# aszepieniec/stark-brainfuck

Hardware: AMD Instinct MI355X
Metric: goldilocks_ntt_field_elements_per_sec (higher is better)
Workload: dtype u64 (mod 2^64-2^32+1)

## Files before the change

### stark_brainfuck_amd/_lib.py

```python
import ctypes
import os

_HERE = os.path.dirname(os.path.abspath(__file__))
LIB_PATH = os.environ.get("BFS_LIB_PATH") or os.path.join(_HERE, "libbfstark_hip.so")

u64 = ctypes.c_uint64
u32 = ctypes.c_uint32
vp = ctypes.c_void_p
sz = ctypes.c_size_t
ci = ctypes.c_int

BFS_OK = 0
ASSERT_CODES = {1, 2, 3, 4, 5, 8, 9}

_SIGNATURES = {
    "bfs_version": (ci, []),
    "bfs_last_error": (ctypes.c_char_p, []),
    "bfs_device_count": (ci, [ctypes.POINTER(ci)]),
    "bfs_set_device": (ci, [ci]),
    "bfs_malloc": (ci, [ctypes.POINTER(vp), sz]),
    "bfs_free": (ci, [vp]),
    "bfs_malloc_async": (ci, [ctypes.POINTER(vp), sz, vp]),
    "bfs_free_async": (ci, [vp, vp]),
    "bfs_pool_trim": (ci, []),
# ... 132 lines not shown
    "bfs_stark_verify_finish": (ci, [vp, vp, ctypes.POINTER(u64), u32, ctypes.POINTER(ci)]),
    "bfs_stark_verify_finish_fri": (ci, [vp, vp, ctypes.POINTER(u64), u32, u32, ci, u32, ctypes.POINTER(ci)]),
    "bfs_stark_session_set_fri": (ci, [vp, u32, ci, u32]),
    "bfs_stark_session_new": (vp, []),
    "bfs_stark_session_free": (None, [vp]),
    "bfs_stark_commit": (ci, [vp, vp, vp, vp, vp, ctypes.POINTER(u64), ctypes.POINTER(u64), ctypes.POINTER(u64), ctypes.POINTER(ctypes.c_double), vp]),
    "bfs_stark_finish": (ci, [vp, vp, ctypes.POINTER(u64), ctypes.POINTER(u64), ctypes.POINTER(u64), u32, ctypes.c_int32, ctypes.POINTER(u64), u32,
                              ctypes.POINTER(u64), vp, ctypes.POINTER(u64), ctypes.POINTER(ctypes.c_double), vp]),
}

_EXT_SIGNATURES = {
    "bfs_poly_eval_points": (ci, [vp, u64, u64, u32, ctypes.POINTER(u64), u32, vp, vp]),
    "bfs_deep_quotient": (ci, [vp, u32, u64, u32, u64, u64, ctypes.POINTER(u64), ctypes.POINTER(u64), u32, ctypes.POINTER(u64), vp, u64, vp]),
}

_OPEN_SIGNATURES = {
    "bfsx_poly_eval_columns": (ci, [vp, u32, ctypes.POINTER(u64), u32, vp, vp]),
    "bfsx_deep_quotient_groups": (ci, [vp, u32, u64, u32, u64, u64, ctypes.POINTER(u32), ctypes.POINTER(u32), u32, ctypes.POINTER(u64), u32,
                                       ctypes.POINTER(u32), ctypes.POINTER(u64), ctypes.POINTER(u64), vp, u64, vp]),
}

_ROUNDS_SIGNATURES = {
    "bfsr_deep_quotient_rounds": (ci, [vp, u32, u64, u32, u64, u64, ctypes.POINTER(u32), ctypes.POINTER(u32), u32, ctypes.POINTER(u64), u32,
                                       ctypes.POINTER(u32), ctypes.POINTER(u64), ctypes.POINTER(u64), vp, u64, ctypes.POINTER(u32), vp]),
}


_COMPOSE_SIGNATURES = {
    "bfsc_air_compose": (ci, [ci, vp, vp, u32, u64, u64, u64, u64, u64, ctypes.POINTER(u64), ctypes.POINTER(u64), ctypes.POINTER(u64), ctypes.POINTER(u64),
                              u32, ci, vp, vp]),
    "bfsc_difference_compose": (ci, [vp, vp, u32, u64, u64, ctypes.POINTER(u64), u32, ci, vp, vp]),
}


class GatherRequest(ctypes.Structure):
    _fields_ = [("d_base", vp), ("nwords", u32), ("stride", u32), ("out_offset", u64)]


class AirViolation(ctypes.Structure):
    _fields_ = [("first_row", u64), ("count", u64)]


class RowColumn(ctypes.Structure):
    _fields_ = [("d_values", vp), ("is_ext", ctypes.c_int32), ("field_id", ctypes.c_int32)]


class EvalColumn(ctypes.Structure):
    _fields_ = [("d_coeffs", vp), ("n_coeffs", u64)]


class TracePadTable(ctypes.Structure):
    _fields_ = [("d_rows", vp), ("rows", u64), ("row_stride", u64), ("height", u64), ("d_out", vp), ("d_mask0", vp), ("d_mask1", vp),
                ("d_mask2", vp), ("kind", ctypes.c_int32), ("width", u32)]


class CombSource(ctypes.Structure):
    _fields_ = [("ptr", vp), ("is_ext", u32), ("pad", u32), ("shift", u64), ("wa", u64 * 3), ("wb", u64 * 3)]

class ScanSpec(ctypes.Structure):
    _fields_ = [("kind", ctypes.c_int32), ("record_before", ctypes.c_int32), ("d_x1", vp), ("d_x2", vp), ("d_x3", vp), ("shift1", u64),
                ("d_mask", vp), ("n", u64), ("constants", u64 * 12), ("initial", u64 * 3), ("d_out", vp), ("out_stride", u64),
                ("d_terminal", vp)]


class StarkParams(ctypes.Structure):
    _fields_ = [("log_n", u32), ("expansion_factor", u32), ("num_colinearity_checks", u32), ("security_level", u32), ("offset", u64),
# ... 14 lines not shown
    _fields_ = [("randomizer_seed", vp), ("randomizer_limbs", vp), ("base_randomizers", vp), ("base_salt_seed", vp), ("base_salts", vp),
                ("initials", u64 * 6), ("ext_randomizers", vp), ("ext_salt_seed", vp), ("ext_salts", vp)]


class CombWeight(ctypes.Structure):
    _fields_ = [("wa", u64 * 3), ("wb", u64 * 3), ("shift", u64)]


_lib = None


class BackendUnavailable(RuntimeError):
    pass


def exported_symbols():
    return sorted(_SIGNATURES)


def ext_exported_symbols():
    return sorted(_EXT_SIGNATURES)


def open_exported_symbols():
    return sorted(_OPEN_SIGNATURES)


def rounds_exported_symbols():
    return sorted(_ROUNDS_SIGNATURES)


def compose_exported_symbols():
    return sorted(_COMPOSE_SIGNATURES)


def load():
    global _lib
    if _lib is not None:
        return _lib
    if not os.path.exists(LIB_PATH):
        raise BackendUnavailable(
            "libbfstark_hip.so is not built (%s). Run `python -m stark_brainfuck_amd.build`; "
            "there is no CPU fallback for the hot path." % LIB_PATH)
    try:
        import torch
    except ImportError:
        pass
    lib = ctypes.CDLL(LIB_PATH)
    for name, (res, args) in (list(_SIGNATURES.items()) + list(_EXT_SIGNATURES.items()) + list(_OPEN_SIGNATURES.items()) + list(_ROUNDS_SIGNATURES.items())
                              + list(_COMPOSE_SIGNATURES.items())):
        fn = getattr(lib, name)
        fn.restype = res
        fn.argtypes = args
    _lib = lib
    return lib


def check(rc):
    if rc == BFS_OK:
        return
    msg = load().bfs_last_error().decode("utf-8", "replace")
    if rc in ASSERT_CODES:
        raise AssertionError(msg)
    raise RuntimeError("libbfstark_hip: error %d: %s" % (rc, msg))
```

### stark_brainfuck_amd/csrc/fri.hip

```cpp
#include <algorithm>
#include <chrono>
#include <map>
#include <unordered_map>
#include <vector>

#include "../../include/bfstark.h"
#include "blake2b.hpp"
#include "refpickle.hpp"
#include "runtime.hpp"

namespace bfs {

template <int K>
__global__ void __launch_bounds__(K == 1 ? 1024 : 256) fri_fold_kernel(FriFoldArgs f, u64* out, u64 out_stride) {
    for (u64 i = (u64)blockIdx.x * blockDim.x + threadIdx.x; i < f.half; i += (u64)gridDim.x * blockDim.x) {
        const Xfe r = fri_fold_point<K>(f, i);
        out[i] = r.c[0];
        out[out_stride + i] = r.c[1];
        out[2 * out_stride + i] = r.c[2];
    }
}

constexpr u32 FRI_FOLD_GRID_MAX = 4096;
static int fri_fold_launch(const FriFoldArgs& f, u64* out, u64 out_stride, hipStream_t stream) {
// ... 19 lines not shown
}

static int gather_run(const std::vector<GatherReq>& reqs, u64 nwords, hipStream_t stream, PinnedLease& req_area, PinnedLease& res_area, const u64** words) {
    BFS_TRY(req_area.get(reqs.size() * sizeof(GatherReq)));
    BFS_TRY(res_area.get(nwords * sizeof(u64)));
    memcpy(req_area.host, reqs.data(), reqs.size() * sizeof(GatherReq));
    hipLaunchKernelGGL(gather_requests_kernel, dim3((u32)((reqs.size() + 255) / 256)), dim3(256), 0, stream, (const GatherReq*)req_area.dev, (u32)reqs.size(),
                       (u64*)res_area.dev);
    BFS_HIP(hipGetLastError());
    BFS_HIP(hipStreamSynchronize(stream));
    *words = (const u64*)res_area.host;
    return BFS_OK;
}

static thread_local double g_fri_timing[8] = {0, 0, 0, 0, 0, 0, 0, 0};
static inline double now_ms() { return std::chrono::duration<double, std::milli>(std::chrono::steady_clock::now().time_since_epoch()).count(); }

enum class TreePath : unsigned char {
    Borrowed,
    Coset,
    OneLaunch,
    FoldInLeaves,
    Codeword,
    SingleElement,
};

struct FriRound {
    const u64* cw = nullptr;
    u64 stride = 0, length = 0;
    u64 leaves = 0;
    u64* nodes = nullptr;
    TreePath path = TreePath::Codeword;
    unsigned char root[64];
};

struct RootMailbox {
    u64* host = nullptr;
    u64* dev = nullptr;
    u64 seq = 0;
    int init() {
        if (host) return BFS_OK;
        BFS_TRY(host_alloc(16 * sizeof(u64), (void**)&host));
        memset(host, 0, 16 * sizeof(u64));
        BFS_HIP(hipHostGetDevicePointer((void**)&dev, host, 0));
        return BFS_OK;
    }
    ~RootMailbox() { if (host) (void)host_release(host); }
};

struct FriSession {
    std::vector<FriRound> rounds;
    void* block = nullptr;
    bool use_workspace = false;
    RootMailbox mailbox;
    u32 log_n = 0;
    u32 log2_folding = 1;
    bool coset_leaves = false;
    u32 grinding_bits = 0;
    u64 grinding_window = POW_DEFAULT_WINDOW;
    u64 round0_leaves = 0;
    struct Key {
        u64 v;
        Key(u32 round, u64 index) : v(((u64)round << 48) | index) {}
        bool operator==(const Key& o) const { return v == o.v; }
    };
    struct KeyMap {
        std::vector<u64> keys;
        std::vector<u32> slots;
        std::vector<rp::Ref> vals;
        void reserve(size_t n) { size_t cap = 64; while (cap < 2 * n) cap <<= 1; if (cap > keys.size()) rehash(cap); vals.reserve(n); }
        void rehash(size_t cap) {
            std::vector<u64> k2(cap, 0);
            std::vector<u32> s2(cap, 0);
            for (size_t i = 0; i < keys.size(); ++i)
                if (keys[i]) { size_t j = slot_of(keys[i], cap); while (k2[j]) j = (j + 1) & (cap - 1); k2[j] = keys[i]; s2[j] = slots[i]; }
            keys.swap(k2); slots.swap(s2);
        }
        static size_t slot_of(u64 stored, size_t cap) { return (size_t)((stored * 0x9E3779B97F4A7C15ULL) >> 20) & (cap - 1); }
        size_t find(const Key& key) const {
            size_t j = slot_of(key.v + 1, keys.size());
// ... 62 lines not shown
        p = (u64*)w;
    } else {
        if (S.block) { (void)device_release(S.block, S.block_stream); S.block = nullptr; }
        BFS_TRY(device_alloc(words * sizeof(u64), stream, &S.block));
        S.block_stream = stream;
        p = (u64*)S.block;
    }
    for (u32 r = 0; r < R; ++r) {
        FriRound& fr = S.rounds[r];
        fr.nodes = p; p += 16 * fr.leaves;
        if (r == 0) { fr.cw = d_cw; fr.stride = stride; }
        else { fr.cw = p; fr.stride = fr.length; p += 3 * fr.length; }
    }
    return S.mailbox.init();
}

static int launch_round_tree(FriSession& S, u32 r, const FriFoldArgs& fold, hipStream_t stream, u64* seq) {
    FriRound& fr = S.rounds[r];
    const bool folds = fold.in != nullptr;
    u64* const cw = (u64*)fr.cw;
    u64* const box = S.mailbox.dev;
    *seq = 0;
    if (folds != (r >= 1)) { set_error("internal: round %u of the plan and its fold disagree", r); return BFS_ERR_BAD_ARG; }
    switch (fr.path) {
    case TreePath::Borrowed:
        fr.nodes = (u64*)S.round0_nodes;
        memcpy(fr.root, S.round0_root, 64);
        return BFS_OK;
    case TreePath::SingleElement:
        if (folds) BFS_TRY(fri_fold_launch(fold, cw, fr.stride, stream));
        return merkle_build_xfe_launch(fr.cw, fr.stride, fr.length, fr.nodes, stream);
    case TreePath::Coset:
        *seq = ++S.mailbox.seq;
        return coset_tree_launch(folds ? &fold : nullptr, cw, fr.stride, fr.leaves, S.log2_folding, fr.nodes, stream, box + 9, *seq, box, *seq);
    case TreePath::OneLaunch:
        *seq = ++S.mailbox.seq;
        return fri_round_fused_launch(fold, cw, fr.stride, fr.length, fr.nodes, stream, box, *seq);
    case TreePath::FoldInLeaves:
        *seq = ++S.mailbox.seq;
        return merkle_build_xfe_fold_launch(fold, cw, fr.stride, fr.length, fr.nodes, stream, box, *seq);
    case TreePath::Codeword:
        *seq = ++S.mailbox.seq;
        return merkle_build_xfe_launch(fr.cw, fr.stride, fr.length, fr.nodes, stream, box, *seq);
    }
    set_error("internal: round %u has no tree path", r);
    return BFS_ERR_BAD_ARG;
}

int fri_commit(FriSession& S, rp::Transcript& ps, const u64* d_cw, u64 stride, u32 log_n, u64 offset, u64 omega,
               u32 expansion, hipStream_t stream) {
    const double t_begin = now_ms();
    BFS_TRY(plan_rounds(S, d_cw, stride, log_n, omega, expansion, stream));
    const u32 k = S.log2_folding;
    const u32 R = (u32)S.rounds.size();
    const u64 *winv_lo = nullptr, *winv_hi = nullptr;
    u32 lo_bits = 0;
    BFS_TRY(ntt_power_tables(gl_inv(omega), log_n, &winv_lo, &winv_hi, &lo_bits));
    u64 g = offset, w = omega;
    FriFoldArgs fold{};
    rp::Transcript::Lookahead look;
    static const bool lookahead_on = getenv("BFS_FRI_LOOKAHEAD") == nullptr || atoi(getenv("BFS_FRI_LOOKAHEAD")) != 0;
    static const bool trace = getenv("BFS_FRI_TRACE") != nullptr;
    bool looking = false, look_begun = false;
    auto begin_lookahead = [&]() {
        if (look_begun) return;
        look_begun = true;
        const double t_look = trace ? now_ms() : 0;
        looking = lookahead_on && R >= 3 && ps.lookahead_begin(look, R - 2);
        if (trace) fprintf(stderr, "fri look-ahead %s: %.1f us, %zu objects in front\n", looking ? "on" : "off", 1e3 * (now_ms() - t_look), ps.objects.size());
    };
    for (u32 r = 0; r < R; ++r) {
        FriRound& fr = S.rounds[r];
        unsigned char seed[32];
        bool have_seed = false, speculating = false;
        const double t_round = trace ? now_ms() : 0;
        double t_launched = 0, t_absorbed = 0, t_root = 0;
        rp::Transcript::Speculation speculation;
        auto await_root = [&](u64 seq) -> int {
            if (trace) t_launched = now_ms();
            if (r >= 1) begin_lookahead();
            if (r + 1 < R) {
                if (r == 0) { ps.fiat_shamir(ps.objects.size(), seed, 32); have_seed = true; }
                else if (!looking) { ps.speculate(speculation); speculating = true; }
            }
            if (trace) t_absorbed = now_ms();
            volatile u64* flag = S.mailbox.host + 8;
            u64 spins = 0;
            while (__atomic_load_n(flag, __ATOMIC_ACQUIRE) != seq) {
                if (++spins > (1ull << 22)) {
                    BFS_HIP(hipStreamSynchronize(stream));
                    if (__atomic_load_n(flag, __ATOMIC_ACQUIRE) != seq) { set_error("root mailbox was not written"); return BFS_ERR_HIP; }
                    break;
                }
            }
            memcpy(fr.root, S.mailbox.host, 64);
            return BFS_OK;
        };
        u64 seq = 0;
        BFS_TRY(launch_round_tree(S, r, fold, stream, &seq));
        if (seq != 0) {
            BFS_TRY(await_root(seq));
            if (fr.path == TreePath::Coset && __atomic_load_n(S.mailbox.host + 9, __ATOMIC_ACQUIRE) == seq) {
                BFS_TRY(coset_tree_rows(fr.cw, fr.stride, fr.leaves, k, fr.nodes, fr.root, stream));
            }
        } else if (fr.path == TreePath::SingleElement) {
            if (r >= 1) begin_lookahead();
            BFS_HIP(hipMemcpyAsync(fr.root, fr.nodes + 8, 64, hipMemcpyDeviceToHost, stream));
            BFS_HIP(hipStreamSynchronize(stream));
        }
        if (trace) t_root = now_ms();
        if (speculating) ps.resolve(speculation, fr.root, seed, 32);
        else if (r > 0 && looking) { ps.lookahead_next(look, fr.root, r + 1 < R ? seed : nullptr, 32); have_seed = r + 1 < R; }
        else if (r > 0) ps.objects.push_back(rp::mk_bytes(fr.root, 64));
        if (trace)
            fprintf(stderr, "fri round %2u  n %8llu  launch %6.1f us  absorb %6.1f us  wait %6.1f us  finish %6.1f us\n", r, (unsigned long long)fr.length,
                    1e3 * (t_launched - t_round), 1e3 * (t_absorbed - t_launched), 1e3 * (t_root - t_absorbed), 1e3 * (now_ms() - t_root));
        if (r == R - 1) break;
        if (!speculating && !have_seed) ps.fiat_shamir(ps.objects.size(), seed, 32);
        fold.in = fr.cw; fold.in_stride = fr.stride;
        fold.winv_lo = winv_lo; fold.winv_hi = winv_hi; fold.lo_bits = lo_bits; fold.round_shift = k * r;
        fri_fold_constants(fold, k, fr.length, rp::sample_xfe(seed, 32), g, w);
        for (u32 j = 0; j < k; ++j) { g = gl_sqr(g); w = gl_sqr(w); }
    }
    g_fri_timing[0] = now_ms() - t_begin;
    FriRound& last = S.rounds[R - 1];
    std::vector<u64> host(3 * last.length);
    if (last.stride == last.length) {
        BFS_HIP(hipMemcpyAsync(host.data(), last.cw, 3 * last.length * sizeof(u64), hipMemcpyDeviceToHost, stream));
    } else {
        for (int k = 0; k < 3; ++k)
            BFS_HIP(hipMemcpyAsync(host.data() + k * last.length, last.cw + k * last.stride, last.length * sizeof(u64), hipMemcpyDeviceToHost, stream));
    }
    BFS_HIP(hipStreamSynchronize(stream));
    std::vector<rp::Ref> items;
    for (u64 j = 0; j < last.length; ++j) {
// ... 480 lines not shown
```

### stark_brainfuck_amd/csrc/merkle.hip

```cpp
#include "blake2b_quad.hpp"
#include "merkle_core.hpp"
#include <vector>

#include "runtime.hpp"

namespace bfs {

constexpr int LEAF_THREADS = 64;

constexpr int LEAF_STAGE_WORDS = XFE_STREAM_WORDS * LEAF_THREADS;

__device__ __forceinline__ void xfe_leaves_wave(u64 c0, u64 c1, u64 c2, bool active, u64* stage , u64 h[8], const u64* midstates) {
    const u32 lane = threadIdx.x;
    const u32 k = active ? xfe_leaf_k(c0, c1, c2) : 0u;
    if (active && k == 0) merkle_leaf_xfe_zero(h, midstates);
    if (__ballot(k == 3) != 0) { if (k == 3) merkle_leaf_xfe_stream<3>(c0, c1, c2, stage + lane, LEAF_THREADS, h, midstates); }
    if (__ballot(k == 2) != 0) { if (k == 2) merkle_leaf_xfe_stream<2>(c0, c1, c2, stage + lane, LEAF_THREADS, h, midstates); }
    if (__ballot(k == 1) != 0) { if (k == 1) merkle_leaf_xfe_stream<1>(c0, c1, c2, stage + lane, LEAF_THREADS, h, midstates); }
}

__device__ __forceinline__ void xfe_leaves_wave_store(u64 c0, u64 c1, u64 c2, bool active, u64* stage, u64* leaf_digests, u64 i, const u64* midstates) {
    u64 d[8];
    xfe_leaves_wave(c0, c1, c2, active, stage, d, midstates);
    if (!active) return;
    u64* out = leaf_digests + i * 8;
#pragma unroll
    for (int j = 0; j < 8; ++j) out[j] = d[j];
}

__global__ void __launch_bounds__(LEAF_THREADS) merkle_leaves_xfe_kernel(const u64* limbs, u64 limb_stride, u64 n, u64* leaf_digests, const u64* midstates) {
    __shared__ u64 stage[LEAF_STAGE_WORDS];
    const u64 i = (u64)blockIdx.x * LEAF_THREADS + threadIdx.x;
    const bool active = i < n;
    u64 c0 = 0, c1 = 0, c2 = 0;
// ... 21 lines not shown

__global__ void __launch_bounds__(LEAF_THREADS) merkle_leaves_bfe_kernel(const u64* values, u64 n, u64* leaf_digests) {
    __shared__ u64 stage[BFE_LEAF_MAX_WORDS * LEAF_THREADS];
    const u64 i = (u64)blockIdx.x * LEAF_THREADS + threadIdx.x;
    if (i >= n) return;
    u64 d[8];
    merkle_leaf_bfe_body(values, i, stage + threadIdx.x, LEAF_THREADS, d);
    u64* out = leaf_digests + i * 8;
#pragma unroll
    for (int j = 0; j < 8; ++j) out[j] = d[j];
}

__global__ void blake2b_batch_kernel(const u64* data, const u64* offsets, const u32* lengths, u64 n, u64* digests) {
    const u64 i = (u64)blockIdx.x * blockDim.x + threadIdx.x;
    if (i >= n) return;
    u64 h[8];
    blake2b_staged<true>(data + offsets[i], 1, lengths[i], h);
    u64* out = digests + i * 8;
#pragma unroll
    for (int j = 0; j < 8; ++j) out[j] = h[j];
}

__global__ void merkle_parents_kernel(u64* nodes, u64 first, u64 count, u64 present_children) {
    const u64 t = (u64)blockIdx.x * blockDim.x + threadIdx.x;
    if (t >= count) return;
    const u64 k = first + t;
    const u64 c = 2 * t;
    int present = c + 1 < present_children ? 2 : (c < present_children ? 1 : 0);
    u64 out[8];
    merkle_parent_body(nodes + (2 * k) * 8, nodes + (2 * k + 1) * 8, present, out);
    u64* dst = nodes + k * 8;
#pragma unroll
    for (int j = 0; j < 8; ++j) dst[j] = out[j];
}

__global__ void __launch_bounds__(256) merkle_top_kernel(u64* nodes, u32 width, u64 present_children, u64* root_out, u64 seq) {
    __shared__ u64 lvl[512 * 8];
    const u32 t = threadIdx.x;
    for (u32 i = t; i < 2 * width * 8; i += 256) lvl[i] = nodes[(u64)2 * width * 8 + i];
    __syncthreads();
    u64 present = present_children;
    for (u32 w = width; w >= 1; w >>= 1) {
        u64 out[8];
        if (t < w) {
            const u64 c = 2 * (u64)t;
            int pr = c + 1 < present ? 2 : (c < present ? 1 : 0);
            merkle_parent_body(lvl + (2 * t) * 8, lvl + (2 * t + 1) * 8, pr, out);
        }
        __syncthreads();
        if (t < w) {
            u64* dst = nodes + ((u64)w + t) * 8;
#pragma unroll
            for (int j = 0; j < 8; ++j) { lvl[t * 8 + j] = out[j]; dst[j] = out[j]; }
            if (w == 1 && root_out != nullptr) {
#pragma unroll
                for (int j = 0; j < 8; ++j) __hip_atomic_store(root_out + j, out[j], __ATOMIC_RELAXED, __HIP_MEMORY_SCOPE_SYSTEM);
                __hip_atomic_store(root_out + 8, seq, __ATOMIC_RELEASE, __HIP_MEMORY_SCOPE_SYSTEM);
            }
        }
        __syncthreads();
        present = 2 * (u64)w;
    }
}


__global__ void __launch_bounds__(256) merkle_parents_quad_kernel(u64* nodes, u64 first, u64 count, u64 present_children) {
#if defined(__HIP_DEVICE_COMPILE__)
    __shared__ u64 msg[64 * 16];
    const u32 q = threadIdx.x >> 2, j = threadIdx.x & 3;
    const u64 t = (u64)blockIdx.x * 64 + q;
    const QuadLane ql = quad_lane(threadIdx.x);
    if (t < count) {
        const u64 k = first + t, c = 2 * t;
        const int present = c + 1 < present_children ? 2 : (c < present_children ? 1 : 0);
        const u64* child = nodes + (2 * k) * 8;
#pragma unroll
        for (int w = 0; w < 4; ++w) {
            const int idx = 4 * j + w;
            msg[q * 16 + idx] = (idx < 8 * present) ? child[idx] : 0;
        }
        u64 hl, hh;
        blake2b_init_quad(ql, hl, hh);
        blake2b_compress_quad(ql, hl, hh, msg + q * 16, (u64)(64 * present + 32 * (2 - present)), true);
        nodes[k * 8 + j] = hl;
        nodes[k * 8 + 4 + j] = hh;
    }
#endif
}

#if defined(__HIP_DEVICE_COMPILE__)
__device__ __forceinline__ void quad_parent(const QuadLane& ql, const u64* m, u64 bytes, u64& hl, u64& hh) {
    blake2b_init_quad(ql, hl, hh);
    blake2b_compress_quad(ql, hl, hh, m, bytes, true);
}
__device__ __forceinline__ void quad_parent_store(u32 j, u64 hl, u64 hh, u64* dst, u64* g) {
    dst[j] = hl;
    dst[4 + j] = hh;
    g[j] = hl;
    g[4 + j] = hh;
}

constexpr int QUAD_LEAF_WORDS = 48;

__device__ __forceinline__ void xfe_leaf_quad(u64 c0, u64 c1, u64 c2, u64* m, const QuadLane& ql, u32 j, const u64* midstates, u64& hl, u64& hh) {
    const u32 k = xfe_leaf_k(c0, c1, c2);
    if (k == 0) {
        hl = midstates[(size_t)2 * LEAF_MS_LEN * 8 + j];
        hh = midstates[(size_t)2 * LEAF_MS_LEN * 8 + 4 + j];
    } else {
        const u32 body = xfe_leaf_body_len(k, c0, c1, c2), total = body + 11;
        const u32 nblk = (total + 127) / 128;
        const u64* ms = midstates + ((size_t)(k == 1 ? 0 : 1) * LEAF_MS_LEN + body) * 8;
        hl = ms[j];
        hh = ms[4 + j];
        if (j == 0) {
            LeafWriter w;
            w.init(m, 1);
            encode_xfe_leaf_tail(w, k, c0, c1, c2);
            for (u32 x = w.wpos; x < (nblk - 1) * 16; ++x) m[x] = 0;
        }
        for (u32 b = 1; b < nblk; ++b) {
            const bool last = b + 1 == nblk;
            blake2b_compress_quad(ql, hl, hh, m + 16 * (b - 1), last ? (u64)total : (u64)(b + 1) * 128, last);
        }
    }
}
#endif

__global__ void __launch_bounds__(1024) merkle_top_quad_kernel(u64* nodes, u32 width, u64 present_children, u64* root_out, u64 seq) {
#if defined(__HIP_DEVICE_COMPILE__)
    __shared__ u64 bufA[512 * 8];
    __shared__ u64 bufB[256 * 8];
    const u32 tid = threadIdx.x, q = tid >> 2, j = tid & 3;
    const QuadLane ql = quad_lane(tid);
    for (u32 i = tid; i < 2 * width * 8; i += 1024) bufA[i] = nodes[(u64)2 * width * 8 + i];
    __syncthreads();
    u64* src = bufA;
    u64* dst = bufB;
    u64 present = present_children;
    for (u32 w = width; w >= 1; w >>= 1) {
        if (q < w) {
            const u64 c = 2 * (u64)q;
            const int pr = c + 1 < present ? 2 : (c < present ? 1 : 0);
            u64* m = src + q * 16;
            if (pr < 2) {
#pragma unroll
                for (int wd = 0; wd < 4; ++wd) { const int idx = 4 * j + wd; if (idx >= 8 * pr) m[idx] = 0; }
            }
            u64 hl, hh;
            quad_parent(ql, m, (u64)(64 * pr + 32 * (2 - pr)), hl, hh);
            quad_parent_store(j, hl, hh, dst + q * 8, nodes + ((u64)w + q) * 8);
            if (w == 1 && root_out != nullptr) {
                __hip_atomic_store(root_out + j, hl, __ATOMIC_RELAXED, __HIP_MEMORY_SCOPE_SYSTEM);
                __hip_atomic_store(root_out + 4 + j, hh, __ATOMIC_RELAXED, __HIP_MEMORY_SCOPE_SYSTEM);
            }
        }
        __syncthreads();
        u64* tmp = src; src = dst; dst = tmp;
        present = 2 * (u64)w;
    }
    if (tid == 0 && root_out != nullptr) {
        __threadfence_system();
        __hip_atomic_store(root_out + 8, seq, __ATOMIC_RELEASE, __HIP_MEMORY_SCOPE_SYSTEM);
    }
#endif
}

__global__ void __launch_bounds__(1024) merkle_subtree_quad_kernel(u64* nodes, u64 children) {
#if defined(__HIP_DEVICE_COMPILE__)
    __shared__ u64 bufA[512 * 8];
    __shared__ u64 bufB[256 * 8];
    const u32 tid = threadIdx.x, q = tid >> 2, j = tid & 3;
    const QuadLane ql = quad_lane(tid);
    const u64* in = nodes + (children + (u64)blockIdx.x * 512) * 8;
    for (u32 i = tid; i < 512 * 8; i += 1024) bufA[i] = in[i];
    __syncthreads();
    u64* src = bufA;
    u64* dst = bufB;
    u64 level = children >> 1;
    for (u32 w = 256; w >= 1; w >>= 1, level >>= 1) {
        if (q < w) {
            u64 hl, hh;
            quad_parent(ql, src + q * 16, 128, hl, hh);
            quad_parent_store(j, hl, hh, dst + q * 8, nodes + (level + (u64)blockIdx.x * w + q) * 8);
        }
        __syncthreads();
        u64* tmp = src; src = dst; dst = tmp;
    }
#endif
}

__global__ void __launch_bounds__(256) merkle_leaves_xfe_quad_kernel(const u64* limbs, u64 limb_stride, u64 n, u64* leaf_digests, const u64* midstates) {
#if defined(__HIP_DEVICE_COMPILE__)
    __shared__ u64 stage[64 * QUAD_LEAF_WORDS];
    const u32 q = threadIdx.x >> 2, j = threadIdx.x & 3;
    const u64 i = (u64)blockIdx.x * 64 + q;
    const QuadLane ql = quad_lane(threadIdx.x);
    if (i >= n) return;
    u64* m = stage + q * QUAD_LEAF_WORDS;
    const u64 c0 = limbs[i], c1 = limbs[limb_stride + i], c2 = limbs[2 * limb_stride + i];
    u64 hl, hh;
    xfe_leaf_quad(c0, c1, c2, m, ql, j, midstates, hl, hh);
    leaf_digests[i * 8 + j] = hl;
    leaf_digests[i * 8 + 4 + j] = hh;
#endif
}

constexpr u32 FRI_WG_LEAVES = 64;

template <int K>
__global__ void __launch_bounds__(4 * FRI_WG_LEAVES) fri_round_quad_kernel(FriFoldArgs f, u64* cw, u64 cw_stride, u64 n, u64* nodes, const u64* midstates,
                                                              u64* root_out, u64 seq) {
#if defined(__HIP_DEVICE_COMPILE__)
    __shared__ u64 stage[FRI_WG_LEAVES * QUAD_LEAF_WORDS];
    __shared__ u64 bufA[FRI_WG_LEAVES * 8];
    __shared__ u64 bufB[FRI_WG_LEAVES * 4];
    __shared__ u64 limbs[3 * FRI_WG_LEAVES];
    const u32 tid = threadIdx.x, q = tid >> 2, j = tid & 3;
    const QuadLane ql = quad_lane(tid);
    const u32 local = n < FRI_WG_LEAVES ? (u32)n : FRI_WG_LEAVES;
    const u64 first = (u64)blockIdx.x * FRI_WG_LEAVES;
    if (tid < local) {
        const u64 i = first + tid;
        u64 c0, c1, c2;
        if (f.in != nullptr) {
            const Xfe r = fri_fold_point<K>(f, i);
            c0 = r.c[0]; c1 = r.c[1]; c2 = r.c[2];
            cw[i] = c0; cw[cw_stride + i] = c1; cw[2 * cw_stride + i] = c2;
        } else {
            c0 = cw[i]; c1 = cw[cw_stride + i]; c2 = cw[2 * cw_stride + i];
        }
        limbs[tid] = c0; limbs[FRI_WG_LEAVES + tid] = c1; limbs[2 * FRI_WG_LEAVES + tid] = c2;
    }
    __syncthreads();
    if (q < local) {
        u64* m = stage + q * QUAD_LEAF_WORDS;
        const u64 c0 = limbs[q], c1 = limbs[FRI_WG_LEAVES + q], c2 = limbs[2 * FRI_WG_LEAVES + q];
        u64 hl, hh;
        xfe_leaf_quad(c0, c1, c2, m, ql, j, midstates, hl, hh);
        u64* g = nodes + (n + first + q) * 8;
        g[j] = hl; g[4 + j] = hh;
        bufA[q * 8 + j] = hl; bufA[q * 8 + 4 + j] = hh;
    }
    __syncthreads();
    u64* src = bufA;
    u64* dst = bufB;
    const u64 groups = n / local;
    const bool whole_tree = groups == 1;
    for (u32 w = local >> 1; w >= 1; w >>= 1) {
        if (q < w) {
            u64 hl, hh;
            quad_parent(ql, src + q * 16, 128, hl, hh);
            quad_parent_store(j, hl, hh, dst + q * 8, nodes + (groups * w + (u64)blockIdx.x * w + q) * 8);
            if (w == 1 && whole_tree && root_out != nullptr) {
                __hip_atomic_store(root_out + j, hl, __ATOMIC_RELAXED, __HIP_MEMORY_SCOPE_SYSTEM);
                __hip_atomic_store(root_out + 4 + j, hh, __ATOMIC_RELAXED, __HIP_MEMORY_SCOPE_SYSTEM);
            }
        }
        __syncthreads();
        u64* tmp = src; src = dst; dst = tmp;
    }
    if (tid == 0 && whole_tree && root_out != nullptr) {
        __threadfence_system();
        __hip_atomic_store(root_out + 8, seq, __ATOMIC_RELEASE, __HIP_MEMORY_SCOPE_SYSTEM);
    }
#endif
}

constexpr u64 QUAD_PARENTS_MAX = 8192;
constexpr u64 SUBTREE_PARENTS_MAX = 65536;
constexpr u64 QUAD_LEAVES_MAX = 8192;

int merkle_inner_launch(u64* d_nodes, u32 depth, u64 n_leaves, hipStream_t stream, u64* root_out, u64 seq) {
    if (depth == 0) return BFS_OK;
    u64 present = n_leaves;
    for (u32 lvl = depth; lvl-- > 0;) {
        const u64 count = 1ull << lvl;
        if (present >= 2 * count && count >= 512 && count <= SUBTREE_PARENTS_MAX) {
            hipLaunchKernelGGL(merkle_subtree_quad_kernel, dim3((u32)(count / 256)), dim3(1024), 0, stream, d_nodes, 2 * count);
            BFS_HIP(hipGetLastError());
            lvl -= 8;
            present = 2 * count;
            continue;
        }
        if (count <= 256) {
            hipLaunchKernelGGL(merkle_top_quad_kernel, dim3(1), dim3(1024), 0, stream, d_nodes, (u32)count, present, root_out, seq);
            BFS_HIP(hipGetLastError());
            return BFS_OK;
        }
        if (count <= QUAD_PARENTS_MAX)
            hipLaunchKernelGGL(merkle_parents_quad_kernel, dim3((u32)((count + 63) / 64)), dim3(256), 0, stream, d_nodes, count, count, present);
        else
            hipLaunchKernelGGL(merkle_parents_kernel, dim3((u32)((count + 255) / 256)), dim3(256), 0, stream, d_nodes, count, count, present);
        BFS_HIP(hipGetLastError());
        present = 2 * count;
    }
    return BFS_OK;
}

static int get_leaf_midstates(const u64** d_table) {
    if (cached_table_lookup(0x6D696473ULL, 1, 0, d_table)) return BFS_OK;
    std::vector<u64> host(LEAF_MS_WORDS);
    leaf_midstates(host.data());
    return cached_table(0x6D696473ULL, 1, 0, host.data(), host.size(), d_table);
}

int merkle_build_xfe_launch(const u64* d_limbs, u64 limb_stride, u64 n, u64* d_nodes, hipStream_t stream, u64* root_out, u64 seq) {
    if (n == 0) return BFS_OK;
    const u64* d_ms = nullptr;
    BFS_TRY(get_leaf_midstates(&d_ms));
    const u32 depth = tree_depth(n);
    const u64 npo2 = 1ull << depth;
    if (n <= QUAD_LEAVES_MAX)
        hipLaunchKernelGGL(merkle_leaves_xfe_quad_kernel, dim3((u32)((n + 63) / 64)), dim3(256), 0, stream, d_limbs, limb_stride, n, d_nodes + npo2 * 8, d_ms);
    else
        hipLaunchKernelGGL(merkle_leaves_xfe_kernel, dim3((u32)((n + LEAF_THREADS - 1) / LEAF_THREADS)), dim3(LEAF_THREADS), 0, stream,
                           d_limbs, limb_stride, n, d_nodes + npo2 * 8, d_ms);
    BFS_HIP(hipGetLastError());
    return merkle_inner_launch(d_nodes, depth, n, stream, root_out, seq);
}

int fri_round_fused_launch(const FriFoldArgs& fold, u64* d_cw, u64 cw_stride, u64 n, u64* d_nodes, hipStream_t stream, u64* root_out, u64 seq) {
    if (n < 2 || n > FRI_FUSED_MAX || (n & (n - 1))) { set_error("internal: fused FRI round on %llu elements", (unsigned long long)n); return BFS_ERR_BAD_ARG; }
    const u64* d_ms = nullptr;
    BFS_TRY(get_leaf_midstates(&d_ms));
    const u32 groups = (u32)(n <= FRI_WG_LEAVES ? 1 : n / FRI_WG_LEAVES);
    const dim3 grid(groups), block(4 * FRI_WG_LEAVES);
    BFS_TRY(with_fold_factor(fold.in == nullptr ? 1u : fold.log2_folding, [&](auto k) -> int {
        hipLaunchKernelGGL(fri_round_quad_kernel<decltype(k)::value>, grid, block, 0, stream, fold, d_cw, cw_stride, n, d_nodes, d_ms, root_out, seq);
        BFS_HIP(hipGetLastError());
        return BFS_OK;
    }));
    if (groups == 1) return BFS_OK;
    return merkle_inner_launch(d_nodes, tree_depth(groups), groups, stream, root_out, seq);
}

int merkle_build_xfe_fold_launch(const FriFoldArgs& fold, u64* d_cw, u64 cw_stride, u64 n, u64* d_nodes, hipStream_t stream, u64* root_out, u64 seq) {
    if (fold.in == nullptr || n <= QUAD_LEAVES_MAX) { set_error("internal: fused fold + leaves on %llu elements", (unsigned long long)n); return BFS_ERR_BAD_ARG; }
    const u64* d_ms = nullptr;
    BFS_TRY(get_leaf_midstates(&d_ms));
    const u32 depth = tree_depth(n);
    const u64 npo2 = 1ull << depth;
    const dim3 grid((u32)((n + LEAF_THREADS - 1) / LEAF_THREADS)), block(LEAF_THREADS);
    BFS_TRY(with_fold_factor(fold.log2_folding, [&](auto k) -> int {
        hipLaunchKernelGGL(merkle_leaves_xfe_fold_kernel<decltype(k)::value>, grid, block, 0, stream, fold, d_cw, cw_stride, n, d_nodes + npo2 * 8, d_ms);
        BFS_HIP(hipGetLastError());
        return BFS_OK;
    }));
    return merkle_inner_launch(d_nodes, depth, n, stream, root_out, seq);
}

int merkle_build_bfe_launch(const u64* d_values, u64 n, u64* d_nodes, hipStream_t stream) {
    if (n == 0) return BFS_OK;
    const u32 depth = tree_depth(n);
    const u64 npo2 = 1ull << depth;
    hipLaunchKernelGGL(merkle_leaves_bfe_kernel, dim3((u32)((n + LEAF_THREADS - 1) / LEAF_THREADS)), dim3(LEAF_THREADS), 0, stream,
                       d_values, n, d_nodes + npo2 * 8);
    BFS_HIP(hipGetLastError());
    return merkle_inner_launch(d_nodes, depth, n, stream);
}

int merkle_build_bytes_launch(const u64* d_data, const u64* d_offsets, const u32* d_lengths, u64 n, u64* d_nodes, hipStream_t stream) {
    if (n == 0) return BFS_OK;
    const u32 depth = tree_depth(n);
    const u64 npo2 = 1ull << depth;
    hipLaunchKernelGGL(blake2b_batch_kernel, dim3((u32)((n + 63) / 64)), dim3(64), 0, stream, d_data, d_offsets, d_lengths, n, d_nodes + npo2 * 8);
    BFS_HIP(hipGetLastError());
    return merkle_inner_launch(d_nodes, depth, n, stream);
}

}
```

### stark_brainfuck_amd/csrc/merkle_core.hpp

```cpp
#pragma once
#include "blake2b.hpp"
#include "leaf_encode.hpp"

namespace bfs {

template <bool MASK_TAIL = false>
BFS_HD void blake2b_staged(const u64* base, u32 stride, u32 total, u64 h[8]) {
    blake2b_init(h);
    const u32 nwords = (total + 7) / 8;
    const u32 nblk = total ? (total + 127) / 128 : 1;
    const u64 tail_mask = (total & 7) ? (~0ull >> (64 - 8 * (total & 7))) : ~0ull;
    for (u32 b = 0; b < nblk; ++b) {
        u64 m[16];
        BFS_UNROLL
        for (int j = 0; j < 16; ++j) {
            u32 w = b * 16 + (u32)j;
            m[j] = w < nwords ? base[(size_t)w * stride] : 0;
            if (MASK_TAIL && w + 1 == nwords) m[j] &= tail_mask;
        }
        const bool last = (b + 1 == nblk);
        blake2b_compress(h, m, last ? (u64)total : (u64)(b + 1) * 128, last);
    }
}

// ... 135 lines not shown
    blake2b_staged(stage, stride, total, h);
    BFS_UNROLL
    for (int j = 0; j < 8; ++j) digest_out[j] = h[j];
}

BFS_HD void load_digest(const u64* p, u64* m) {
#if defined(__HIP_DEVICE_COMPILE__)
    typedef u64 u64x2 __attribute__((ext_vector_type(2)));
    const u64x2* q = (const u64x2*)p;
    BFS_UNROLL
    for (int j = 0; j < 4; ++j) {
        const u64x2 v = q[j];
        m[2 * j] = v.x;
        m[2 * j + 1] = v.y;
    }
#else
    for (int j = 0; j < 8; ++j) m[j] = p[j];
#endif
}

BFS_HD void merkle_parent_body(const u64* left, const u64* right, int present, u64* out) {
    u64 m[16];
    BFS_UNROLL
    for (int j = 0; j < 16; ++j) m[j] = 0;
    if (present >= 1) load_digest(left, m);
    if (present >= 2) load_digest(right, m + 8);
    u64 h[8];
    blake2b_init(h);
    blake2b_compress(h, m, (u64)(64 * present + 32 * (2 - present)), true);
    BFS_UNROLL
    for (int j = 0; j < 8; ++j) out[j] = h[j];
}

}
```

### stark_brainfuck_amd/csrc/runtime.hpp

```cpp
#pragma once
#include <hip/hip_runtime.h>
#include <stddef.h>
#include <stdint.h>

#include <type_traits>

#include "ntt_plan.hpp"

namespace bfs {

void set_error(const char* fmt, ...) __attribute__((format(printf, 1, 2)));
const char* last_error();

#define BFS_HIP(expr)                                                                                   \
    do {                                                                                                \
        hipError_t e_ = (expr);                                                                         \
        if (e_ != hipSuccess) {                                                                         \
            ::bfs::set_error("%s failed: %s (%s:%d)", #expr, hipGetErrorString(e_), __FILE__, __LINE__); \
            return BFS_ERR_HIP;                                                                         \
        }                                                                                               \
    } while (0)

#define BFS_TRY(expr)            \
    do {                         \
// ... 108 lines not shown
    hipStream_t stream;
};
constexpr u64 NTT_STREAMING_BYTES = 128ull << 20;
int ntt_launch(const u64* d_in, u64 n_in, u64 in_stride, u64* d_out, u64 out_stride, u32 log_n, u32 batch, u64 root,
               u64 shift, u64 post_scale, hipStream_t stream);
int ntt_run_steps(const NttCall& c, const NttPlan& p, u64* mid, u32 first, u32 last);
int ntt_power_tables(u64 root, u32 log_n, const u64** lo, const u64** hi, u32* lo_bits);
constexpr int NTT_ROUTE_CANDIDATES = 3;
constexpr int NTT_ROUTE_DIRECT = -1;
enum class NttRouteMode { Remembered, Auto, Forced };
struct NttEnv {
    NttRouteMode route_mode;
    int forced_route;
    bool probe_log;
    int force_streaming;
    bool allow_expand;
    bool plan_log;
};
const NttEnv& ntt_env();

constexpr int NTT_ROUTE_SLOT0 = 16;
int ntt_route(const NttCall& c, const NttPlan& p, int* route);
int ntt_route_probe_info(float* us, int* route, unsigned long long* probes);
int ntt_tune(const u64* d_in, u64 in_stride, u64* d_out, u64 out_stride, u32 log_n, u32 batch, u64 root, hipStream_t stream, int* route_out);
size_t ntt_route_forget_range(const void* lo, size_t bytes, bool may_free);
void ntt_route_trim();

int mul_pointwise_launch(const u64* a, const u64* b, u64* out, u64 n, hipStream_t stream);
int batch_inverse_launch(const u64* in, u64* out, u64 n, hipStream_t stream);
int scale_launch(const u64* in, u64* out, u64 n, u64 stride, u32 batch, u64 factor, hipStream_t stream);
int xfe_mul_pointwise_launch(const u64* a, u64 a_stride, const u64* b, u64 b_stride, u64* out, u64 out_stride, u64 n, hipStream_t stream);
int xfe_batch_inverse_launch(const u64* in, u64 in_stride, u64* out, u64 out_stride, u64 n, hipStream_t stream);

int merkle_inner_launch(u64* d_nodes, u32 depth, u64 n_leaves, hipStream_t stream, u64* root_out = nullptr, u64 seq = 0);
int merkle_build_xfe_launch(const u64* d_limbs, u64 limb_stride, u64 n, u64* d_nodes, hipStream_t stream, u64* root_out = nullptr, u64 seq = 0);
int merkle_build_bfe_launch(const u64* d_values, u64 n, u64* d_nodes, hipStream_t stream);
int merkle_build_bytes_launch(const u64* d_data, const u64* d_offsets, const u32* d_lengths, u64 n, u64* d_nodes, hipStream_t stream);

int coset_tree_launch(const FriFoldArgs* fold, u64* d_cw, u64 cw_stride, u64 q, u32 log2_coset, u64* d_nodes, hipStream_t stream, u64* not_mine,
                      u64 token, u64* root_out, u64 seq);
int coset_tree_rows(const u64* d_cw, u64 cw_stride, u64 q, u32 log2_coset, u64* d_nodes, unsigned char h_root[64], hipStream_t stream);

constexpr u64 POW_DEFAULT_WINDOW = 1ULL << 24;
int pow_search(const u64 seed[4], u32 bits, u64 first, u64 count, u64* nonce, bool* found, hipStream_t stream);

struct PinnedLease {
    void* host = nullptr;
    void* dev = nullptr;
    int get(size_t need) {
        BFS_TRY(host_alloc(need < 4096 ? 4096 : need, &host));
        BFS_HIP(hipHostGetDevicePointer(&dev, host, 0));
        return BFS_OK;
    }
    ~PinnedLease() { if (host) (void)host_release(host); }
    PinnedLease() = default;
    PinnedLease(const PinnedLease&) = delete;
    PinnedLease& operator=(const PinnedLease&) = delete;
};

}
```

Baseline: 103.8 billion.

## Publish a Merkle level to host mailbox and finish the top on CPU

```diff
diff --git a/include/bfstark_tops.h b/include/bfstark_tops.h
--- /dev/null
+++ b/include/bfstark_tops.h
@@ -0,0 +1,20 @@
+#ifndef BFSTARK_TOPS_H
+#define BFSTARK_TOPS_H
+
+#include "bfstark.h"
+
+#ifdef __cplusplus
+extern "C" {
+#endif
+
+int bfst_merkle_top_host(const uint8_t* h_nodes, uint32_t count, uint8_t h_root[64]);
+
+int bfst_tree_host_levels(void);
+
+int bfst_tree_host_levels_set(int levels);
+
+#ifdef __cplusplus
+}
+#endif
+
+#endif
diff --git a/stark_brainfuck_amd/_lib.py b/stark_brainfuck_amd/_lib.py
--- a/stark_brainfuck_amd/_lib.py
+++ b/stark_brainfuck_amd/_lib.py
@@ -188,6 +188,12 @@
     "bfsc_difference_compose": (ci, [vp, vp, u32, u64, u64, ctypes.POINTER(u64), u32, ci, vp, vp]),
 }
 
+_TOPS_SIGNATURES = {
+    "bfst_merkle_top_host": (ci, [ctypes.c_char_p, u32, vp]),
+    "bfst_tree_host_levels": (ci, []),
+    "bfst_tree_host_levels_set": (ci, [ci]),
+}
+
 
 class GatherRequest(ctypes.Structure):
     _fields_ = [("d_base", vp), ("nwords", u32), ("stride", u32), ("out_offset", u64)]
@@ -268,6 +274,10 @@
 
 def compose_exported_symbols():
     return sorted(_COMPOSE_SIGNATURES)
+
+
+def tops_exported_symbols():
+    return sorted(_TOPS_SIGNATURES)
 
 
 def load():
@@ -284,7 +294,7 @@
         pass
     lib = ctypes.CDLL(LIB_PATH)
     for name, (res, args) in (list(_SIGNATURES.items()) + list(_EXT_SIGNATURES.items()) + list(_OPEN_SIGNATURES.items()) + list(_ROUNDS_SIGNATURES.items())
-                              + list(_COMPOSE_SIGNATURES.items())):
+                              + list(_COMPOSE_SIGNATURES.items()) + list(_TOPS_SIGNATURES.items())):
         fn = getattr(lib, name)
         fn.restype = res
         fn.argtypes = args
diff --git a/stark_brainfuck_amd/csrc/fri.hip b/stark_brainfuck_amd/csrc/fri.hip
--- a/stark_brainfuck_amd/csrc/fri.hip
+++ b/stark_brainfuck_amd/csrc/fri.hip
@@ -75,20 +75,6 @@
     u64* nodes = nullptr;
     TreePath path = TreePath::Codeword;
     unsigned char root[64];
-};
-
-struct RootMailbox {
-    u64* host = nullptr;
-    u64* dev = nullptr;
-    u64 seq = 0;
-    int init() {
-        if (host) return BFS_OK;
-        BFS_TRY(host_alloc(16 * sizeof(u64), (void**)&host));
-        memset(host, 0, 16 * sizeof(u64));
-        BFS_HIP(hipHostGetDevicePointer((void**)&dev, host, 0));
-        return BFS_OK;
-    }
-    ~RootMailbox() { if (host) (void)host_release(host); }
 };
 
 struct FriSession {
@@ -217,7 +203,7 @@
         return merkle_build_xfe_launch(fr.cw, fr.stride, fr.length, fr.nodes, stream);
     case TreePath::Coset:
         *seq = ++S.mailbox.seq;
-        return coset_tree_launch(folds ? &fold : nullptr, cw, fr.stride, fr.leaves, S.log2_folding, fr.nodes, stream, box + 9, *seq, box, *seq);
+        return coset_tree_launch(folds ? &fold : nullptr, cw, fr.stride, fr.leaves, S.log2_folding, fr.nodes, stream, box + MAILBOX_TOKEN, *seq, box, *seq);
     case TreePath::OneLaunch:
         *seq = ++S.mailbox.seq;
         return fri_round_fused_launch(fold, cw, fr.stride, fr.length, fr.nodes, stream, box, *seq);
@@ -269,23 +255,13 @@
                 else if (!looking) { ps.speculate(speculation); speculating = true; }
             }
             if (trace) t_absorbed = now_ms();
-            volatile u64* flag = S.mailbox.host + 8;
-            u64 spins = 0;
-            while (__atomic_load_n(flag, __ATOMIC_ACQUIRE) != seq) {
-                if (++spins > (1ull << 22)) {
-                    BFS_HIP(hipStreamSynchronize(stream));
-                    if (__atomic_load_n(flag, __ATOMIC_ACQUIRE) != seq) { set_error("root mailbox was not written"); return BFS_ERR_HIP; }
-                    break;
-                }
-            }
-            memcpy(fr.root, S.mailbox.host, 64);
-            return BFS_OK;
+            return mailbox_await_root(S.mailbox, seq, fr.leaves, stream, fr.root);
         };
         u64 seq = 0;
         BFS_TRY(launch_round_tree(S, r, fold, stream, &seq));
         if (seq != 0) {
             BFS_TRY(await_root(seq));
-            if (fr.path == TreePath::Coset && __atomic_load_n(S.mailbox.host + 9, __ATOMIC_ACQUIRE) == seq) {
+            if (fr.path == TreePath::Coset && __atomic_load_n(S.mailbox.host + MAILBOX_TOKEN, __ATOMIC_ACQUIRE) == seq) {
                 BFS_TRY(coset_tree_rows(fr.cw, fr.stride, fr.leaves, k, fr.nodes, fr.root, stream));
             }
         } else if (fr.path == TreePath::SingleElement) {
diff --git a/stark_brainfuck_amd/csrc/merkle.hip b/stark_brainfuck_amd/csrc/merkle.hip
--- a/stark_brainfuck_amd/csrc/merkle.hip
+++ b/stark_brainfuck_amd/csrc/merkle.hip
@@ -1,5 +1,7 @@
 #include "blake2b_quad.hpp"
 #include "merkle_core.hpp"
+#include <atomic>
+#include <cstdlib>
 #include <vector>
 
 #include "runtime.hpp"
@@ -87,35 +89,6 @@
     u64* dst = nodes + k * 8;
 #pragma unroll
     for (int j = 0; j < 8; ++j) dst[j] = out[j];
-}
-
-__global__ void __launch_bounds__(256) merkle_top_kernel(u64* nodes, u32 width, u64 present_children, u64* root_out, u64 seq) {
-    __shared__ u64 lvl[512 * 8];
-    const u32 t = threadIdx.x;
-    for (u32 i = t; i < 2 * width * 8; i += 256) lvl[i] = nodes[(u64)2 * width * 8 + i];
-    __syncthreads();
-    u64 present = present_children;
-    for (u32 w = width; w >= 1; w >>= 1) {
-        u64 out[8];
-        if (t < w) {
-            const u64 c = 2 * (u64)t;
-            int pr = c + 1 < present ? 2 : (c < present ? 1 : 0);
-            merkle_parent_body(lvl + (2 * t) * 8, lvl + (2 * t + 1) * 8, pr, out);
-        }
-        __syncthreads();
-        if (t < w) {
-            u64* dst = nodes + ((u64)w + t) * 8;
-#pragma unroll
-            for (int j = 0; j < 8; ++j) { lvl[t * 8 + j] = out[j]; dst[j] = out[j]; }
-            if (w == 1 && root_out != nullptr) {
-#pragma unroll
-                for (int j = 0; j < 8; ++j) __hip_atomic_store(root_out + j, out[j], __ATOMIC_RELAXED, __HIP_MEMORY_SCOPE_SYSTEM);
-                __hip_atomic_store(root_out + 8, seq, __ATOMIC_RELEASE, __HIP_MEMORY_SCOPE_SYSTEM);
-            }
-        }
-        __syncthreads();
-        present = 2 * (u64)w;
-    }
 }
 
 
@@ -182,7 +155,18 @@
 }
 #endif
 
-__global__ void __launch_bounds__(1024) merkle_top_quad_kernel(u64* nodes, u32 width, u64 present_children, u64* root_out, u64 seq) {
+__device__ __forceinline__ void publish_digest(u64* root_out, u32 node, u32 j, u64 hl, u64 hh) {
+    u64* at = root_out + MAILBOX_LEVEL + node * 8;
+    __hip_atomic_store(at + j, hl, __ATOMIC_RELAXED, __HIP_MEMORY_SCOPE_SYSTEM);
+    __hip_atomic_store(at + 4 + j, hh, __ATOMIC_RELAXED, __HIP_MEMORY_SCOPE_SYSTEM);
+    __threadfence_system();
+}
+__device__ __forceinline__ void publish_flag(u64* root_out, u32 count, u64 seq) {
+    __hip_atomic_store(root_out + MAILBOX_COUNT, (u64)count, __ATOMIC_RELAXED, __HIP_MEMORY_SCOPE_SYSTEM);
+    __hip_atomic_store(root_out + MAILBOX_FLAG, seq, __ATOMIC_RELEASE, __HIP_MEMORY_SCOPE_SYSTEM);
+}
+
+__global__ void __launch_bounds__(1024) merkle_top_quad_kernel(u64* nodes, u32 width, u64 present_children, u64* root_out, u64 seq, u32 publish) {
 #if defined(__HIP_DEVICE_COMPILE__)
     __shared__ u64 bufA[512 * 8];
     __shared__ u64 bufB[256 * 8];
@@ -190,10 +174,17 @@
     const QuadLane ql = quad_lane(tid);
     for (u32 i = tid; i < 2 * width * 8; i += 1024) bufA[i] = nodes[(u64)2 * width * 8 + i];
     __syncthreads();
+    const bool publish_input = root_out != nullptr && 2 * width <= publish;
+    if (publish_input) {
+        if (q < 2 * width) publish_digest(root_out, q, j, bufA[q * 8 + j], bufA[q * 8 + 4 + j]);
+        __syncthreads();
+        if (tid == 0) publish_flag(root_out, 2 * width, seq);
+    }
     u64* src = bufA;
     u64* dst = bufB;
     u64 present = present_children;
     for (u32 w = width; w >= 1; w >>= 1) {
+        const bool publish_level = root_out != nullptr && !publish_input && w == publish;
         if (q < w) {
             const u64 c = 2 * (u64)q;
             const int pr = c + 1 < present ? 2 : (c < present ? 1 : 0);
@@ -205,18 +196,12 @@
             u64 hl, hh;
             quad_parent(ql, m, (u64)(64 * pr + 32 * (2 - pr)), hl, hh);
             quad_parent_store(j, hl, hh, dst + q * 8, nodes + ((u64)w + q) * 8);
-            if (w == 1 && root_out != nullptr) {
-                __hip_atomic_store(root_out + j, hl, __ATOMIC_RELAXED, __HIP_MEMORY_SCOPE_SYSTEM);
-                __hip_atomic_store(root_out + 4 + j, hh, __ATOMIC_RELAXED, __HIP_MEMORY_SCOPE_SYSTEM);
-            }
+            if (publish_level) publish_digest(root_out, q, j, hl, hh);
         }
         __syncthreads();
+        if (publish_level && tid == 0) publish_flag(root_out, w, seq);
         u64* tmp = src; src = dst; dst = tmp;
         present = 2 * (u64)w;
-    }
-    if (tid == 0 && root_out != nullptr) {
-        __threadfence_system();
-        __hip_atomic_store(root_out + 8, seq, __ATOMIC_RELEASE, __HIP_MEMORY_SCOPE_SYSTEM);
     }
 #endif
 }
@@ -265,7 +250,7 @@
 
 template <int K>
 __global__ void __launch_bounds__(4 * FRI_WG_LEAVES) fri_round_quad_kernel(FriFoldArgs f, u64* cw, u64 cw_stride, u64 n, u64* nodes, const u64* midstates,
-                                                              u64* root_out, u64 seq) {
+                                                              u64* root_out, u64 seq, u32 publish) {
 #if defined(__HIP_DEVICE_COMPILE__)
     __shared__ u64 stage[FRI_WG_LEAVES * QUAD_LEAF_WORDS];
     __shared__ u64 bufA[FRI_WG_LEAVES * 8];
@@ -288,6 +273,9 @@
         limbs[tid] = c0; limbs[FRI_WG_LEAVES + tid] = c1; limbs[2 * FRI_WG_LEAVES + tid] = c2;
     }
     __syncthreads();
+    const u64 groups = n / local;
+    const bool publishes = groups == 1 && root_out != nullptr;
+    const bool publish_leaves = publishes && local <= publish;
     if (q < local) {
         u64* m = stage + q * QUAD_LEAF_WORDS;
         const u64 c0 = limbs[q], c1 = limbs[FRI_WG_LEAVES + q], c2 = limbs[2 * FRI_WG_LEAVES + q];
@@ -296,28 +284,23 @@
         u64* g = nodes + (n + first + q) * 8;
         g[j] = hl; g[4 + j] = hh;
         bufA[q * 8 + j] = hl; bufA[q * 8 + 4 + j] = hh;
+        if (publish_leaves) publish_digest(root_out, q, j, hl, hh);
     }
     __syncthreads();
+    if (publish_leaves && tid == 0) publish_flag(root_out, local, seq);
     u64* src = bufA;
     u64* dst = bufB;
-    const u64 groups = n / local;
-    const bool whole_tree = groups == 1;
     for (u32 w = local >> 1; w >= 1; w >>= 1) {
+        const bool publish_level = publishes && !publish_leaves && w == publish;
         if (q < w) {
             u64 hl, hh;
             quad_parent(ql, src + q * 16, 128, hl, hh);
             quad_parent_store(j, hl, hh, dst + q * 8, nodes + (groups * w + (u64)blockIdx.x * w + q) * 8);
-            if (w == 1 && whole_tree && root_out != nullptr) {
-                __hip_atomic_store(root_out + j, hl, __ATOMIC_RELAXED, __HIP_MEMORY_SCOPE_SYSTEM);
-                __hip_atomic_store(root_out + 4 + j, hh, __ATOMIC_RELAXED, __HIP_MEMORY_SCOPE_SYSTEM);
-            }
+            if (publish_level) publish_digest(root_out, q, j, hl, hh);
         }
         __syncthreads();
+        if (publish_level && tid == 0) publish_flag(root_out, w, seq);
         u64* tmp = src; src = dst; dst = tmp;
-    }
-    if (tid == 0 && whole_tree && root_out != nullptr) {
-        __threadfence_system();
-        __hip_atomic_store(root_out + 8, seq, __ATOMIC_RELEASE, __HIP_MEMORY_SCOPE_SYSTEM);
     }
 #endif
 }
@@ -325,6 +308,44 @@
 constexpr u64 QUAD_PARENTS_MAX = 8192;
 constexpr u64 SUBTREE_PARENTS_MAX = 65536;
 constexpr u64 QUAD_LEAVES_MAX = 8192;
+
+static std::atomic<int> g_tree_host_levels{-1};
+static int tree_host_levels_default() {
+    const char* e = getenv("BFS_TREE_HOST_LEVELS");
+    const int k = e && *e ? atoi(e) : BFS_TREE_HOST_LEVELS_DEFAULT;
+    return k < 0 ? 0 : (k > MERKLE_HOST_LEVELS_MAX ? MERKLE_HOST_LEVELS_MAX : k);
+}
+int tree_host_levels() {
+    int k = g_tree_host_levels.load(std::memory_order_relaxed);
+    if (k < 0) { k = tree_host_levels_default(); g_tree_host_levels.store(k, std::memory_order_relaxed); }
+    return k;
+}
+int tree_host_levels_set(int levels) {
+    const int before = tree_host_levels();
+    g_tree_host_levels.store(levels < 0 ? tree_host_levels_default() : (levels > MERKLE_HOST_LEVELS_MAX ? MERKLE_HOST_LEVELS_MAX : levels), std::memory_order_relaxed);
+    return before;
+}
+static u32 publish_nodes() { return 1u << tree_host_levels(); }
+
+int mailbox_await_root(RootMailbox& box, u64 seq, u64 leaves, hipStream_t stream, unsigned char root[64]) {
+    volatile u64* flag = box.host + MAILBOX_FLAG;
+    u64 spins = 0;
+    while (__atomic_load_n(flag, __ATOMIC_ACQUIRE) != seq) {
+        if (++spins > (1ull << 22)) {
+            BFS_HIP(hipStreamSynchronize(stream));
+            if (__atomic_load_n(flag, __ATOMIC_ACQUIRE) != seq) { set_error("root mailbox was not written"); return BFS_ERR_HIP; }
+            break;
+        }
+    }
+    const u64 count = __atomic_load_n(box.host + MAILBOX_COUNT, __ATOMIC_RELAXED);
+    u64 top[8];
+    if (count > leaves || !merkle_top_host(box.host + MAILBOX_LEVEL, (u32)(count > MERKLE_HOST_TOP_MAX ? 0 : count), top)) {
+        set_error("internal: a tree of %llu leaves published a level of %llu nodes", (unsigned long long)leaves, (unsigned long long)count);
+        return BFS_ERR_BAD_ARG;
+    }
+    memcpy(root, top, 64);
+    return BFS_OK;
+}
 
 int merkle_inner_launch(u64* d_nodes, u32 depth, u64 n_leaves, hipStream_t stream, u64* root_out, u64 seq) {
     if (depth == 0) return BFS_OK;
@@ -339,7 +360,7 @@
             continue;
         }
         if (count <= 256) {
-            hipLaunchKernelGGL(merkle_top_quad_kernel, dim3(1), dim3(1024), 0, stream, d_nodes, (u32)count, present, root_out, seq);
+            hipLaunchKernelGGL(merkle_top_quad_kernel, dim3(1), dim3(1024), 0, stream, d_nodes, (u32)count, present, root_out, seq, publish_nodes());
             BFS_HIP(hipGetLastError());
             return BFS_OK;
         }
@@ -382,7 +403,7 @@
     const u32 groups = (u32)(n <= FRI_WG_LEAVES ? 1 : n / FRI_WG_LEAVES);
     const dim3 grid(groups), block(4 * FRI_WG_LEAVES);
     BFS_TRY(with_fold_factor(fold.in == nullptr ? 1u : fold.log2_folding, [&](auto k) -> int {
-        hipLaunchKernelGGL(fri_round_quad_kernel<decltype(k)::value>, grid, block, 0, stream, fold, d_cw, cw_stride, n, d_nodes, d_ms, root_out, seq);
+        hipLaunchKernelGGL(fri_round_quad_kernel<decltype(k)::value>, grid, block, 0, stream, fold, d_cw, cw_stride, n, d_nodes, d_ms, root_out, seq, publish_nodes());
         BFS_HIP(hipGetLastError());
         return BFS_OK;
     }));
@@ -425,3 +446,22 @@
 }
 
 }
+
+#include "../../include/bfstark_tops.h"
+extern "C" {
+
+int bfst_merkle_top_host(const uint8_t* h_nodes, uint32_t count, uint8_t h_root[64]) {
+    bfs::u64 lvl[bfs::MERKLE_HOST_TOP_MAX * 8], root[8];
+    if (count >= 1 && count <= bfs::MERKLE_HOST_TOP_MAX) memcpy(lvl, h_nodes, (size_t)count * 64);
+    if (!bfs::merkle_top_host(lvl, count, root)) {
+        bfs::set_error("bfst_merkle_top_host: a level of %u nodes (a power of two in 1 .. %u)", count, bfs::MERKLE_HOST_TOP_MAX);
+        return BFS_ERR_BAD_ARG;
+    }
+    memcpy(h_root, root, 64);
+    return BFS_OK;
+}
+
+int bfst_tree_host_levels(void) { return bfs::tree_host_levels(); }
+int bfst_tree_host_levels_set(int levels) { return bfs::tree_host_levels_set(levels); }
+
+}
diff --git a/stark_brainfuck_amd/csrc/merkle_core.hpp b/stark_brainfuck_amd/csrc/merkle_core.hpp
--- a/stark_brainfuck_amd/csrc/merkle_core.hpp
+++ b/stark_brainfuck_amd/csrc/merkle_core.hpp
@@ -191,4 +191,20 @@
     for (int j = 0; j < 8; ++j) out[j] = h[j];
 }
 
-}
+constexpr u32 MERKLE_HOST_TOP_MAX = 64;
+constexpr int MERKLE_HOST_LEVELS_MAX = 6;
+inline bool merkle_top_host(const u64* nodes, u32 count, u64 root[8]) {
+    if (count == 0 || count > MERKLE_HOST_TOP_MAX || (count & (count - 1))) return false;
+    u64 lvl[MERKLE_HOST_TOP_MAX * 8];
+    memcpy(lvl, nodes, (size_t)count * 64);
+    for (u32 w = count >> 1; w >= 1; w >>= 1)
+        for (u32 i = 0; i < w; ++i) {
+            unsigned char d[64];
+            blake2b_host(lvl + 16 * i, 128, d);
+            memcpy(lvl + 8 * i, d, 64);
+        }
+    memcpy(root, lvl, 64);
+    return true;
+}
+
+}
diff --git a/stark_brainfuck_amd/csrc/runtime.hpp b/stark_brainfuck_amd/csrc/runtime.hpp
--- a/stark_brainfuck_amd/csrc/runtime.hpp
+++ b/stark_brainfuck_amd/csrc/runtime.hpp
@@ -164,6 +164,27 @@
 int xfe_mul_pointwise_launch(const u64* a, u64 a_stride, const u64* b, u64 b_stride, u64* out, u64 out_stride, u64 n, hipStream_t stream);
 int xfe_batch_inverse_launch(const u64* in, u64 in_stride, u64* out, u64 out_stride, u64 n, hipStream_t stream);
 
+constexpr u32 MAILBOX_FLAG = 8, MAILBOX_TOKEN = 9, MAILBOX_COUNT = 10, MAILBOX_LEVEL = 16;
+constexpr u32 MAILBOX_WORDS = MAILBOX_LEVEL + 64 * 8;
+#ifndef BFS_TREE_HOST_LEVELS_DEFAULT
+#define BFS_TREE_HOST_LEVELS_DEFAULT 4
+#endif
+int tree_host_levels();
+int tree_host_levels_set(int levels);
+struct RootMailbox {
+    u64* host = nullptr;
+    u64* dev = nullptr;
+    u64 seq = 0;
+    int init() {
+        if (host) return BFS_OK;
+        BFS_TRY(host_alloc(MAILBOX_WORDS * sizeof(u64), (void**)&host));
+        for (u32 i = 0; i < MAILBOX_WORDS; ++i) host[i] = 0;
+        BFS_HIP(hipHostGetDevicePointer((void**)&dev, host, 0));
+        return BFS_OK;
+    }
+    ~RootMailbox() { if (host) (void)host_release(host); }
+};
+int mailbox_await_root(RootMailbox& box, u64 seq, u64 leaves, hipStream_t stream, unsigned char root[64]);
 int merkle_inner_launch(u64* d_nodes, u32 depth, u64 n_leaves, hipStream_t stream, u64* root_out = nullptr, u64 seq = 0);
 int merkle_build_xfe_launch(const u64* d_limbs, u64 limb_stride, u64 n, u64* d_nodes, hipStream_t stream, u64* root_out = nullptr, u64 seq = 0);
 int merkle_build_bfe_launch(const u64* d_values, u64 n, u64* d_nodes, hipStream_t stream);
```

Result: no change. 103.7 billion (-0.0%).
